# Ecogenomics/CheckM

Measured on NVIDIA H100. Metric: genomes/hour, higher is better.
Workload: dtype int16 (SSV) / u8 (MSV) / int16 (Viterbi) / f32 (Forward, domain definition)

## Files before the change

### checkm_b200/csrc/kernels_vitp.cu

```cuda
#include "engine.hpp"
#include "device_utils.cuh"
#include "stages.hpp"

namespace ckm {

constexpr uint32_t VP_FLOORW = 0xD800D800u;
constexpr int      VP_FLOOR  = -10240;
constexpr uint32_t VP_TFLOORW = 0xC000C000u;

__device__ __forceinline__ int vp_lo(uint32_t w) { return (int)(int16_t)(w & 0xffffu); }
__device__ __forceinline__ int vp_hi(uint32_t w) { return (int)w >> 16; }

template <int W, bool TSMEM>
__global__ void __launch_bounds__(128) vitp_kernel(FilterParams p, int cls) {
  extern __shared__ __align__(16) uint8_t vsm[];
  const int lane = threadIdx.x & 31, warp = threadIdx.x >> 5, wpb = blockDim.x >> 5;
  uint4 *tws = reinterpret_cast<uint4 *>(vsm) + (size_t)warp * W * 64;
  const uint32_t sel = (lane == 0) ? 0x1054u : 0x3210u;
  const int n = min(*p.in_count, p.in_cap);
  int32_t *cursor = (p.vit_work != nullptr) ? p.vit_work + cls : nullptr;
  for (int64_t it = 0;; ++it) {
    int64_t base64;
    if (cursor != nullptr) {
      int b = 0;
      if (lane == 0) b = atomicAdd(cursor, 32);
      base64 = __shfl_sync(0xffffffffu, b, 0);
    } else {
      base64 = ((it * gridDim.x + blockIdx.x) * wpb + warp) * 32;
    }
    if (base64 >= n) break;
    const int base = (int)base64;
    bool mine = false;
    if (base + lane < n) {
      const int vq = p.ms[p.in[base + lane].model].vq;
      mine = (vq == 2 * W) || (W == 1 && vq == 0);
    }
    unsigned todo = __ballot_sync(0xffffffffu, mine);
  while (todo != 0u) {
    const int c = base + __ffs(todo) - 1;
    todo &= todo - 1u;
    Candidate cd = p.in[c];
    const int m = cd.model;
    const ModelScalars ms = p.ms[m];
    const bool unclassed = (ms.vq == 0 && W == 1);
    if (ms.vq != 2 * W && !unclassed) continue;
    const int s = cd.seq, L = p.len[s];
    bool pass = true, redo = false;
    if (cd.P > p.F2) {
      const int tmove = p.tmove_w[s];
      const int cost = -tmove - (int)ms.vit_tbm + 64;
      const bool c1 = (cost - (int)ms.xw_e_loop <= 22528) && (cost <= 22240);
      const bool c1p = (cost - (int)ms.xw_e_loop <= 16384);
      redo = unclassed || !c1;
      float vsc = 0.0f;
      if (!redo) {
        uint4 tr0[TSMEM ? 1 : W], tr1[TSMEM ? 1 : W];
        const uint4 *tsrc = p.twp + ms.blk_off * 32;
        if (TSMEM) {
          __syncwarp();
          for (int z = lane; z < W * 64; z += 32) tws[(z & 1) * (W * 32) + (z >> 1)] = __ldg(tsrc + z);
          __syncwarp();
        } else {
#pragma unroll
          for (int w = 0; w < W; ++w) { tr0[TSMEM ? 0 : w] = __ldg(tsrc + (w * 32 + lane) * 2); tr1[TSMEM ? 0 : w] = __ldg(tsrc + (w * 32 + lane) * 2 + 1); }
        }
#define TR0(w) (TSMEM ? tws[(w) * 32 + lane] : tr0[TSMEM ? 0 : (w)])
#define TR1(w) (TSMEM ? tws[W * 32 + (w) * 32 + lane] : tr1[TSMEM ? 0 : (w)])
        const uint32_t *rwp = p.rwp + ms.blk_off * 32 * (KPAD / 2) + lane;
        uint32_t Mx[W], Ix[W], Dx[W];
#pragma unroll
        for (int w = 0; w < W; ++w) { Mx[w] = VP_FLOORW; Ix[w] = VP_FLOORW; Dx[w] = VP_FLOORW; }
        const int ddbound = ms.ddbound_w, cap = 32767 - (int)ms.vit_emax;
        const int e_move = ms.xw_e_move, e_loop = ms.xw_e_loop;
        int xN = ms.base_w, xB = xN + tmove, xJ = -32768, xC = -32768;
        const uint4 *rp = reinterpret_cast<const uint4 *>(p.res + p.off[s]);
        const int nblk = (L + 15) >> 4;
        uint4 r16 = (nblk > 0) ? __ldg(rp) : make_uint4(0, 0, 0, 0);
        uint32_t ecur[W];
        {
          const uint32_t x0 = r16.x & 0xffu;
#pragma unroll
          for (int w = 0; w < W; ++w) ecur[w] = __ldg(rwp + (x0 * W + w) * 32);
        }
        bool stop = false;
        for (int b = 0; b < nblk && !stop; ++b) {
          const uint4 rnext = (b + 1 < nblk) ? __ldg(rp + b + 1) : make_uint4(0, 0, 0, 0);
          for (int j = 0; j < 4 && !stop; ++j) {
            const uint32_t wcur = (j == 0) ? r16.x : (j == 1) ? r16.y : (j == 2) ? r16.z : r16.w;
            const uint32_t wnxt = (j == 0) ? r16.y : (j == 1) ? r16.z : (j == 2) ? r16.w : rnext.x;
#pragma unroll
            for (int rr = 0; rr < 4; ++rr) {
              if (b * 16 + j * 4 + rr >= L) { stop = true; break; }
              uint32_t enext[W];
              {
                const uint32_t xn = (rr < 3) ? ((wcur >> (8 * (rr + 1))) & 0xffu) : (wnxt & 0xffu);
#pragma unroll
                for (int w = 0; w < W; ++w) enext[w] = __ldg(rwp + (xn * W + w) * 32);
              }
              const uint32_t shM = __shfl_sync(0xffffffffu, Mx[W - 1], (lane + 31) & 31);
              const uint32_t shI = __shfl_sync(0xffffffffu, Ix[W - 1], (lane + 31) & 31);
              const uint32_t shD = __shfl_sync(0xffffffffu, Dx[W - 1], (lane + 31) & 31);
              const uint32_t pm0 = __byte_perm(shM, VP_FLOORW, sel), pi0 = __byte_perm(shI, VP_FLOORW, sel), pd0 = __byte_perm(shD, VP_FLOORW, sel);
              const uint32_t xBw = __byte_perm((uint32_t)xB, 0u, 0x1010u);
              uint32_t md[W];
              uint32_t xEw = VP_FLOORW, dmw = VP_FLOORW;
#pragma unroll
              for (int w = W - 1; w >= 0; --w) {
                const uint32_t pm = (w > 0) ? Mx[w - 1] : pm0, pi = (w > 0) ? Ix[w - 1] : pi0, pd = (w > 0) ? Dx[w - 1] : pd0;
                const uint4 t0 = TR0(w), t1 = TR1(w);
                uint32_t sv = __viaddmax_s16x2(xBw, t0.x, VP_FLOORW);
                sv = __viaddmax_s16x2(pm, t0.y, sv);
                sv = __viaddmax_s16x2(pi, t0.z, sv);
                sv = __viaddmax_s16x2(pd, t0.w, sv);
                sv = __viaddmax_s16x2(sv, ecur[w], VP_FLOORW);
                const uint32_t nI = __viaddmax_s16x2(Ix[w], t1.z, __viaddmax_s16x2(Mx[w], t1.y, VP_FLOORW));
                md[w] = __viaddmax_s16x2(sv, t1.x, VP_FLOORW);
                Mx[w] = sv; Ix[w] = nI;
              }
#pragma unroll
              for (int w = 0; w + 1 < W; w += 2) { xEw = __vimax3_s16x2(xEw, Mx[w], Mx[w + 1]); dmw = __vimax3_s16x2(dmw, md[w], md[w + 1]); }
              if (W & 1) { xEw = __vimax3_s16x2(xEw, Mx[W - 1], Mx[W - 1]); dmw = __vimax3_s16x2(dmw, md[W - 1], md[W - 1]); }
              const int xE = __reduce_max_sync(0xffffffffu, max(vp_lo(xEw), vp_hi(xEw)));
              if (xE >= cap) { redo = true; stop = true; break; }
              xC = max(xC, xE + e_move);
              xJ = max(xJ, xE + e_loop);
              xB = max(xJ + tmove, xN + tmove);
              const int Dmax = __reduce_max_sync(0xffffffffu, max(vp_lo(dmw), vp_hi(dmw)));
              if (Dmax + ddbound > xB) {
                if (!c1p) { redo = true; stop = true; break; }
                uint32_t Bb = VP_FLOORW, Tb = 0u;
#pragma unroll
                for (int w = 0; w < W; ++w) { const uint32_t tdd = TR1(w).w; Bb = __viaddmax_s16x2(Bb, tdd, md[w]); Tb = __viaddmax_s16x2(Tb, __vimax3_s16x2(tdd, VP_TFLOORW, VP_TFLOORW), VP_TFLOORW); }
                uint32_t Bs = Bb, Ts = Tb;
#pragma unroll
                for (int o = 1; o < 32; o <<= 1) {
                  const uint32_t Bl = __shfl_up_sync(0xffffffffu, Bs, o), Tl = __shfl_up_sync(0xffffffffu, Ts, o);
                  if (lane >= o) { Bs = __viaddmax_s16x2(Bl, Ts, Bs); Ts = __viaddmax_s16x2(Ts, Tl, VP_TFLOORW); }
                }
                uint32_t din = __shfl_up_sync(0xffffffffu, Bs, 1), Tex = __shfl_up_sync(0xffffffffu, Ts, 1);
                if (lane == 0) { din = VP_FLOORW; Tex = 0u; }
                const uint32_t lowexit = __shfl_sync(0xffffffffu, Bs, 31);
                const uint32_t dmid = __byte_perm(lowexit, VP_FLOORW, 0x1054u);
                din = __viaddmax_s16x2(dmid, Tex, din);
                uint32_t d = din;
#pragma unroll
                for (int w = 0; w < W; ++w) { Dx[w] = d; d = __viaddmax_s16x2(d, TR1(w).w, md[w]); }
              } else {
                const uint32_t shd = __shfl_sync(0xffffffffu, md[W - 1], (lane + 31) & 31);
#pragma unroll
                for (int w = W - 1; w >= 1; --w) Dx[w] = md[w - 1];
                Dx[0] = __byte_perm(shd, VP_FLOORW, sel);
              }
#pragma unroll
              for (int w = 0; w < W; ++w) ecur[w] = enext[w];
            }
          }
          r16 = rnext;
        }
        if (!redo && xC <= VP_FLOOR + e_move) redo = true;
        if (!redo) {
          vsc = __fsub_rn(__fadd_rn((float)xC, (float)tmove), (float)ms.base_w);
          vsc = __fdiv_rn(vsc, ms.scale_w);
          vsc = __fsub_rn(vsc, 3.0f);
        }
#undef TR0
#undef TR1
      }
      if (redo) {
        if (lane == 0) {
          const int pos = atomicAdd(p.redo_count, 1);
          if (pos < p.redo_cap) p.redo[pos] = cd;
        }
        continue;
      }
      cd.vitsc = vsc;
      const float seq_score = __fdiv_rn(__fsub_rn(vsc, cd.filtersc), 0.69314718055994529f);
      const double P = gumbel_surv((double)seq_score, (double)ms.evparam[2], (double)ms.evparam[3]);
      cd.P = P;
      pass = (P <= p.F2);
      if (lane == 0 && p.dense_vit != nullptr) p.dense_vit[(int64_t)p.model_slot[m] * p.nseq + s] = vsc;
    }
    if (lane == 0 && pass) {
      const int pos = atomicAdd(p.out_count, 1);
      if (pos < p.out_cap) p.out[pos] = cd;
      if (p.dense_passed != nullptr) atomicOr_u8(p.dense_passed, (int64_t)p.model_slot[m] * p.nseq + s, 4);
    }
  }
  }
}

template <int W, bool TSMEM>
static int launch_vitp_w(const FilterParams &p, int cls, int grid, cudaStream_t st) {
  const int sm = TSMEM ? 4 * W * 64 * (int)sizeof(uint4) : 0;
  if (sm > 48 * 1024) {
    cudaError_t e = cudaFuncSetAttribute(vitp_kernel<W, TSMEM>, cudaFuncAttributeMaxDynamicSharedMemorySize, sm);
    if (e != cudaSuccess) return cuda_fail(e, "cudaFuncSetAttribute(vitp)");
  }
  vitp_kernel<W, TSMEM><<<grid, 128, sm, st>>>(p, cls);
  cudaError_t e = cudaGetLastError();
  return e == cudaSuccess ? CKM_OK : cuda_fail(e, "vitp_kernel launch");
}

__global__ void all_pairs_kernel(Candidate *out, int32_t *count, const int32_t *slot_model, int32_t nslots, int32_t nseq) {
  const int64_t n = (int64_t)nslots * nseq;
  for (int64_t i = blockIdx.x * (int64_t)blockDim.x + threadIdx.x; i < n; i += (int64_t)gridDim.x * blockDim.x) {
    Candidate cd;
    cd.seq = (int32_t)(i % nseq); cd.model = slot_model[i / nseq]; cd.usc = 0.0f; cd.filtersc = 0.0f; cd.vitsc = 0.0f; cd.fwdsc = 0.0f; cd.P = 1.0;
    out[i] = cd;
  }
  if (blockIdx.x == 0 && threadIdx.x == 0) *count = (int32_t)n;
}
int launch_all_pairs(Candidate *out, int32_t *count, const int32_t *slot_model, int32_t nslots, int32_t nseq, cudaStream_t st) {
  all_pairs_kernel<<<592, 256, 0, st>>>(out, count, slot_model, nslots, nseq);
  cudaError_t e = cudaGetLastError();
  return e == cudaSuccess ? CKM_OK : cuda_fail(e, "all_pairs_kernel launch");
}

int launch_vitp(const FilterParams &p, int cls, int grid, cudaStream_t st) {
  switch (cls) {
    case 0: return launch_vitp_w<1, false>(p, cls, grid, st);
    case 1: return launch_vitp_w<2, false>(p, cls, grid, st);
    case 2: return launch_vitp_w<3, false>(p, cls, grid, st);
    case 3: return launch_vitp_w<4, false>(p, cls, grid, st);
    case 4: return launch_vitp_w<6, true>(p, cls, grid, st);
    case 5: return launch_vitp_w<8, true>(p, cls, grid, st);
    case 6: return launch_vitp_w<10, true>(p, cls, grid, st);
    case 7: return launch_vitp_w<12, true>(p, cls, grid, st);
    case 8: return launch_vitp_w<14, true>(p, cls, grid, st);
    case 9: return launch_vitp_w<16, true>(p, cls, grid, st);
  }
  set_error("launch_vitp: bad class"); return CKM_EINVAL;
// ... 4 lines not shown
```

### checkm_b200/csrc/search.cu

```cuda
#include <algorithm>
#include <atomic>
#include <chrono>
#include <cstdio>
#include <cmath>
#include <cstdlib>
#include <cstring>
#include <memory>
#include <vector>
#include "engine.hpp"
#include "stages.hpp"
#include "pool.hpp"

using namespace ckm;

namespace ckm {

std::atomic<int> g_live_engines{0};
thread_local ckm_engine *g_pool_engine = nullptr;
thread_local int g_pool_next = 0;
constexpr int X_NX_HOST = 6;
struct EnsembleJob;
int ensembles_launch(ckm_engine *e, const ckm_models *m, DomdefParams &p, const std::vector<PairWork> &pairs,
                     const std::vector<Region> &regs, const std::vector<int> &multi_idx, const std::vector<EnsembleCaps> &caps,
                     cudaStream_t st, EnsembleJob **job_out);
// ... 230 lines not shown
  for (int c = 0; c < 4; ++c) {
    if (gl[c].empty() || db->nseq == 0) continue;
    sp.group_list = s1.glist.as<int32_t>() + goff[c]; sp.ngroups = (int32_t)gl[c].size();
    sp.unit_counter = e->d_counters + CTR_UNIT4 + c;
    int64_t maxbytes = 0;
    for (int g : gl[c]) maxbytes = std::max<int64_t>(maxbytes, m->groups[g].table_bytes);
    const int64_t units = (int64_t)sp.ngroups * sp.nchunks;
    const int grid = (int)std::min<int64_t>(nsm, units);
    if ((rc = launch_ssv(Js[c], sp, grid, (size_t)maxbytes, st))) return rc;
    e->stats.kernel_launches++;
  }
  if (!m->ssv_bypass.empty()) {
    if ((rc = launch_ssv_bypass(m->d_ssv_bypass, (int32_t)m->ssv_bypass.size(), db->nseq, db->d_len, db->d_bin,
                                am.all_active ? nullptr : am.model_active.as<uint8_t>(), (int32_t)m->models.size(),
                                s1.cand.as<int2>(), e->d_counters + CTR_CAND, s1.cand_cap, st))) return rc;
    e->stats.kernel_launches++;
  }
  CKM_CUDA(cudaEventRecord(e->ev[EV_MSV], st));
  MsvParams p{};
  p.res = db->d_res; p.off = db->d_off; p.len = db->d_len; p.nullsc = db->d_nullsc; p.tjb = db->d_tjb;
  p.ms = m->d_scalars; p.rbv = m->d_rbv; p.rmb = m->d_rmb;
  p.cand = s1.cand.as<int2>(); p.cand_count = e->d_counters + CTR_CAND; p.cand_cap = s1.cand_cap;
  p.out = s1.pass.as<Candidate>(); p.out_count = e->d_counters + CTR_MSV; p.out_cap = s1.pass_cap;
  p.xj_dense = xj_dense; p.model_slot = am.model_slot.as<int32_t>(); p.nseq = db->nseq;
  p.row_bytes = (m->maxM + 2 + 15) / 16 * 16;
  p.F1 = 0.02;
  p.use_blk = k.blk ? 1 : 0;
  if ((rc = per_class(e, p, launch_msv2, 16, launch_msv_exact, 4))) return rc;
  e->stats.kernel_launches += 1 + (p.use_blk ? N_BLK_CLASSES : 0);
  CKM_CUDA(cudaEventRecord(e->ev[EV_BIAS], st));
  return CKM_OK;
}

static int run_viterbi(ckm_engine *e, FilterParams &p, bool packed) {
  int rc;
  if (packed) {
    p.vit_work = e->d_counters + CTR_VWORK;
    if ((rc = per_class<FilterParams>(e, p, launch_vitp, 8, nullptr, 0))) return rc;
    p.in = p.redo; p.in_count = p.redo_count; p.in_cap = p.redo_cap;
  }
  return per_class(e, p, launch_vit2, 8, launch_vit, 4);
}
struct Stage2 {
  DevBuf a, b, redo;
  int32_t cap = 0;
};
static int run_stage2(ckm_engine *e, const SearchKnobs &k, const ckm_models *m, const ckm_seqdb *db, ActiveMasks &am, Stage1 &s1, Stage2 &s2,
                      float *d_filtersc, float *d_vit, float *d_fwd, uint8_t *d_passed) {
  cudaStream_t st = e->stream;
  int rc;
  s2.cap = s1.pass_cap;
  if ((rc = s2.a.alloc(sizeof(Candidate) * (size_t)s2.cap))) return rc;
  if ((rc = s2.b.alloc(sizeof(Candidate) * (size_t)s2.cap))) return rc;
  if ((rc = s2.redo.alloc(sizeof(Candidate) * (size_t)s2.cap))) return rc;
  const int nsm = e->prop.multiProcessorCount;
  FilterParams p = filter_params(m, db, am);
  p.redo = s2.redo.as<Candidate>(); p.redo_count = e->d_counters + CTR_VREDO; p.redo_cap = s2.cap;
  p.use_blk = k.blk ? 1 : 0;
  p.dense_filtersc = d_filtersc; p.dense_vit = d_vit; p.dense_fwd = d_fwd; p.dense_passed = d_passed;
  p.in = s1.pass.as<Candidate>(); p.in_count = e->d_counters + CTR_MSV; p.in_cap = s1.pass_cap;
  p.out = s2.a.as<Candidate>(); p.out_count = e->d_counters + CTR_BIAS; p.out_cap = s2.cap;
  if ((rc = launch_bias(p, nsm * 8, st))) return rc;
  CKM_CUDA(cudaEventRecord(e->ev[EV_VIT], st));
  p.in = s2.a.as<Candidate>(); p.in_count = e->d_counters + CTR_BIAS; p.in_cap = s2.cap;
  p.out = s2.b.as<Candidate>(); p.out_count = e->d_counters + CTR_VIT; p.out_cap = s2.cap;
  if ((rc = run_viterbi(e, p, k.vitp))) return rc;
  CKM_CUDA(cudaEventRecord(e->ev[EV_FWD], st));
  p.in = s2.b.as<Candidate>(); p.in_count = e->d_counters + CTR_VIT; p.in_cap = s2.cap;
  p.out = s2.a.as<Candidate>(); p.out_count = e->d_counters + CTR_FWD; p.out_cap = s2.cap;
  if ((rc = per_class(e, p, launch_fwd2, 8, launch_fwd, 4, true))) return rc;
  CKM_CUDA(cudaEventRecord(e->ev[EV_CASCADE_END], st));
  e->stats.kernel_launches += 3 + (k.vitp ? N_BLK_CLASSES : 0) + (p.use_blk ? 2 * N_BLK_CLASSES : 0);
  return CKM_OK;
}

static int64_t envelope_need(const ckm_models *m, const PairWork &pw, const Envelope &en, bool use_blk) {
  const int64_t Ld = en.j - en.i + 1, Mpad = ((m->models[pw.model].M + 1) + 31) / 32 * 32 + 32;
  const int64_t vq = use_blk ? vq_of(m->models[pw.model].M) : 0;
  const int64_t width = vq ? 32 * vq : Mpad;
  return (vq ? 1 : 2) * (Ld + 1) * 3 * width + (Ld + 1) * 15 + 64;
}
static int run_envelope_waves(ckm_engine *e, const ckm_models *m, const std::vector<PairWork> &pairs, DomdefParams &p, int64_t budget,
                              DevBuf &scratch, std::vector<Envelope> &ev, DevBuf &d_ev, DevBuf &d_ord, bool leave_last) {
  if (ev.empty()) return CKM_OK;
  cudaStream_t st = e->stream;
  int rc;
  std::vector<int64_t> need(ev.size());
  std::vector<int8_t> ecls(ev.size());
  for (size_t i = 0; i < ev.size(); ++i) {
    const PairWork &pw = pairs[ev[i].pair];
    need[i] = envelope_need(m, pw, ev[i], p.use_blk != 0);
    ecls[i] = (int8_t)cls_of(m->models[pw.model].M, p.use_blk != 0);
  }
  budget = std::max<int64_t>(budget, *std::max_element(need.begin(), need.end()));
  if ((rc = d_ev.alloc(sizeof(Envelope) * ev.size())) || (rc = d_ord.alloc(sizeof(int32_t) * ev.size()))) return rc;
  std::vector<int32_t> eorder(ev.size());
  for (size_t w0 = 0, w1; w0 < ev.size(); w0 = w1) {
    int64_t tot = 0;
    for (w1 = w0; w1 < ev.size() && (w1 == w0 || tot + need[w1] <= budget); ++w1) { ev[w1].scratch_off = tot; tot += need[w1]; }
// ... 451 lines not shown
  if ((rc = run_stage1(e, k, m, db, q.am, n, s1, nullptr))) return rc;
  if ((rc = run_stage2(e, k, m, db, q.am, s1, s2, dfs.as<float>(), dvit.as<float>(), dfwd.as<float>(), dpass.as<uint8_t>()))) return rc;
  int32_t ctr[CTR_N];
  CKM_CUDA(cudaMemcpyAsync(ctr, e->d_counters, sizeof(ctr), cudaMemcpyDeviceToHost, e->stream));
  CKM_CUDA(cudaMemcpyAsync(filtersc_out, dfs.p, sizeof(float) * (size_t)n, cudaMemcpyDeviceToHost, e->stream));
  CKM_CUDA(cudaMemcpyAsync(vit_out, dvit.p, sizeof(float) * (size_t)n, cudaMemcpyDeviceToHost, e->stream));
  CKM_CUDA(cudaMemcpyAsync(fwd_out, dfwd.p, sizeof(float) * (size_t)n, cudaMemcpyDeviceToHost, e->stream));
  CKM_CUDA(cudaMemcpyAsync(passed_out, dpass.p, (size_t)n, cudaMemcpyDeviceToHost, e->stream));
  CKM_CUDA(cudaStreamSynchronize(e->stream));
  if (ctr[CTR_CAND] > s1.cand_cap || ctr[CTR_MSV] > s1.pass_cap) { set_error("candidate queue overflow"); return CKM_ECAPACITY; }
  std::vector<Candidate> pass1((size_t)ctr[CTR_MSV]);
  if (!pass1.empty()) CKM_CUDA(cudaMemcpy(pass1.data(), s1.pass.p, sizeof(Candidate) * pass1.size(), cudaMemcpyDeviceToHost));
  for (const Candidate &c : pass1) passed_out[(int64_t)q.qorder[0][c.model] * db->nseq + c.seq] |= 1;
  fill_filter_stats(e, n, ctr,  0, 5);
  return CKM_OK;
}

int ckm_viterbi_scores(ckm_engine *e, const ckm_models *m, const int32_t *model_idx, int32_t nmodels,
                       const ckm_seqdb *db, int32_t mode, float *vit_out) {
  if (!e || !m || !db || !vit_out) { set_error("ckm_viterbi_scores: bad argument"); return CKM_EINVAL; }
  cudaSetDevice(e->device);
  cudaStream_t st = e->stream;
  const int ndb = (int)m->models.size();
  if (model_idx == nullptr) nmodels = ndb;
  const int64_t n = (int64_t)nmodels * db->nseq;
  if (n > ((int64_t)1 << 30)) { set_error("ckm_viterbi_scores: too many pairs for one call"); return CKM_ECAPACITY; }
  PoolScope pool_scope(e);
  ActiveMasks am; std::vector<int32_t> slot;
  int rc = build_masks(m, db, model_idx, nmodels, nullptr, am, slot, st);
  if (rc) return rc;
  std::vector<int32_t> slot_model((size_t)std::max(nmodels, 1));
  for (int i = 0; i < nmodels; ++i) slot_model[i] = model_idx ? model_idx[i] : i;
  const size_t nf = (size_t)std::max<int64_t>(n, 1);
  DevBuf dsm, din, dout, dredo, dvit;
  if ((rc = dsm.alloc(sizeof(int32_t) * slot_model.size())) || (rc = din.alloc(sizeof(Candidate) * nf)) || (rc = dout.alloc(sizeof(Candidate) * nf)) ||
      (rc = dredo.alloc(sizeof(Candidate) * nf)) || (rc = dvit.alloc(sizeof(float) * nf))) return rc;
  CKM_CUDA(cudaMemcpyAsync(dsm.p, slot_model.data(), sizeof(int32_t) * slot_model.size(), cudaMemcpyHostToDevice, st));
  CKM_CUDA(cudaMemsetAsync(e->d_counters, 0, CTR_N * sizeof(int32_t), st));
  CKM_CUDA(cudaMemsetAsync(dvit.p, 0xff, sizeof(float) * nf, st));
  std::memset(&e->stats, 0, sizeof(e->stats));
  if (n > 0) {
    if ((rc = launch_all_pairs(din.as<Candidate>(), e->d_counters + CTR_BIAS, dsm.as<int32_t>(), nmodels, db->nseq, st))) return rc;
    FilterParams p = filter_params(m, db, am);
    p.use_blk = (mode == 2) ? 0 : 1;
    p.dense_vit = dvit.as<float>();
    p.redo = dredo.as<Candidate>(); p.redo_count = e->d_counters + CTR_VREDO; p.redo_cap = (int32_t)nf;
    p.in = din.as<Candidate>(); p.in_count = e->d_counters + CTR_BIAS; p.in_cap = (int32_t)nf;
    p.out = dout.as<Candidate>(); p.out_count = e->d_counters + CTR_VIT; p.out_cap = (int32_t)nf;
    if ((rc = run_viterbi(e, p, mode == 0))) return rc;
  }
  int32_t ctr[CTR_N];
  CKM_CUDA(cudaMemcpyAsync(ctr, e->d_counters, sizeof(ctr), cudaMemcpyDeviceToHost, st));
  CKM_CUDA(cudaMemcpyAsync(vit_out, dvit.p, sizeof(float) * (size_t)n, cudaMemcpyDeviceToHost, st));
  CKM_CUDA(cudaStreamSynchronize(st));
  e->stats.n_pairs = n; e->stats.n_past_bias = ctr[CTR_BIAS]; e->stats.n_past_vit = ctr[CTR_VIT]; e->stats.n_vit_redo = ctr[CTR_VREDO];
  return CKM_OK;
}

int ckm_msv_scores(ckm_engine *e, const ckm_models *m, const int32_t *model_idx, int32_t nmodels,
                   const ckm_seqdb *db, int32_t *xj_out) {
  if (!e || !m || !db || !xj_out) { set_error("ckm_msv_scores: bad argument"); return CKM_EINVAL; }
  cudaSetDevice(e->device);
  const SearchKnobs k = read_knobs(false);
  PoolScope pool_scope(e);
  QueryPlan q;
  int rc = plan_queries(m, db, model_idx, nmodels, nullptr, q, e->stream);
  if (rc) return rc;
  const int64_t n = q.n_pairs;
  DevBuf dense;
  if ((rc = dense.alloc(sizeof(int32_t) * (size_t)std::max<int64_t>(n, 1)))) return rc;
  CKM_CUDA(cudaMemsetAsync(dense.p, 0xff, sizeof(int32_t) * (size_t)n, e->stream));
  Stage1 s1;
  std::memset(&e->stats, 0, sizeof(e->stats));
  if ((rc = run_stage1(e, k, m, db, q.am, n, s1, dense.as<int32_t>()))) return rc;
  int32_t ctr[CTR_N];
  CKM_CUDA(cudaMemcpyAsync(ctr, e->d_counters, sizeof(ctr), cudaMemcpyDeviceToHost, e->stream));
  unsigned long long cells = 0;
  CKM_CUDA(cudaMemcpyAsync(&cells, s1.cells.p, sizeof(cells), cudaMemcpyDeviceToHost, e->stream));
  CKM_CUDA(cudaMemcpyAsync(xj_out, dense.p, sizeof(int32_t) * (size_t)n, cudaMemcpyDeviceToHost, e->stream));
  CKM_CUDA(cudaStreamSynchronize(e->stream));
  if (ctr[CTR_CAND] > s1.cand_cap || ctr[CTR_MSV] > s1.pass_cap) { set_error("candidate queue overflow"); return CKM_ECAPACITY; }
  fill_filter_stats(e, n, ctr, cells, 2);
// ... 5 lines not shown
```

### checkm_b200/csrc/stages.hpp

```cpp
#pragma once
#include "engine.hpp"

namespace ckm {

#ifndef CKM_SSV_WARPS
#define CKM_SSV_WARPS 16
#endif
constexpr int SSV_WARPS = CKM_SSV_WARPS;
constexpr int SSV_WARPS_HOST = SSV_WARPS;
constexpr int MSV_WARPS = 8;

struct SsvParams {
  const uint8_t *res; const int64_t *off; const int32_t *len; const int32_t *bin;
  const float *msvB; const int32_t *tjb; const int32_t *order;
  int32_t nseq, seq_chunk, nchunks;
  const TileGroup *groups; const int32_t *group_list; int32_t ngroups;
  const TileDesc *tiles; const TileModel *tile_models;
  const int32_t *chain_first_tile, *chain_ntiles;
  const uint8_t *tile_blob;
  const uint8_t *tile_active;
  const uint8_t *model_active;
  int32_t ntiles, nmodels;
  int32_t *unit_counter;
  int2 *cand; int32_t *cand_count; int32_t cand_cap;
// ... 10 lines not shown
int launch_ssv(int J, const SsvParams &p, int grid, size_t smem_bytes, cudaStream_t stream);

struct MsvParams {
  const uint8_t *res; const int64_t *off; const int32_t *len;
  const float *nullsc; const int32_t *tjb;
  const ModelScalars *ms; const uint8_t *rbv; const uint32_t *rmb;
  const int2 *cand; const int32_t *cand_count; int32_t cand_cap;
  Candidate *out; int32_t *out_count; int32_t out_cap;
  int32_t *xj_dense;
  const int32_t *model_slot;
  int32_t nseq;
  int32_t row_bytes;
  int32_t use_blk;
  double F1;
};

int launch_msv_exact(const MsvParams &p, int grid, cudaStream_t stream);
int launch_ssv_bypass(const int32_t *models, int32_t nbypass, int32_t nseq, const int32_t *len, const int32_t *bin,
                      const uint8_t *model_active, int32_t nmodels_db, int2 *cand, int32_t *cand_count, int32_t cand_cap,
                      cudaStream_t stream);
int launch_msv2(const MsvParams &p, int cls, int grid, cudaStream_t stream);

constexpr int VIT_WARPS = 4;
constexpr int FWD_WARPS = 4;
struct FilterParams {
  const uint8_t *res; const int64_t *off; const int32_t *len;
  const float *lenA, *lenB;
  const int16_t *tmove_w;
  const ModelScalars *ms;
  const float *bias_eo; const int16_t *rwv; const int16_t *twv; const float *rfv; const float *tfv;
  const uint4 *twb; const uint32_t *rwb; const float4 *tfb; const float *rfb;
  const uint4 *twp; const uint32_t *rwp;
  Candidate *redo; int32_t *redo_count; int32_t redo_cap;
  int32_t *vit_work;
  const Candidate *in; const int32_t *in_count; int32_t in_cap;
  Candidate *out; int32_t *out_count; int32_t out_cap;
  int32_t row_elems;
  double F1, F2, F3;
  int32_t use_blk;
  float *dense_filtersc, *dense_vit, *dense_fwd; uint8_t *dense_passed;
  const int32_t *model_slot; int32_t nseq;
};
int launch_bias(const FilterParams &p, int grid, cudaStream_t st);
int launch_vit(const FilterParams &p, int grid, cudaStream_t st);
constexpr int N_BLK_CLASSES = 10;
constexpr int BLK_Q[N_BLK_CLASSES] = {2, 4, 6, 8, 12, 16, 20, 24, 28, 32};
int launch_vit2(const FilterParams &p, int cls, int grid, cudaStream_t st);
int launch_vitp(const FilterParams &p, int cls, int grid, cudaStream_t st);
int launch_all_pairs(Candidate *out, int32_t *count, const int32_t *slot_model, int32_t nslots, int32_t nseq, cudaStream_t st);
int launch_fwd(const FilterParams &p, int grid, cudaStream_t st);

#define FLT_MIN_F 1.17549435e-38f
struct PairWork {
  int32_t seq, model, L;
  int32_t first_dom, ndom_slots;
  float   fwdsc, filtersc, usc;
  int64_t row_off;
};
struct Region { int32_t pair, i, j, multi; };
constexpr int ENS_MAXENV = 32;
struct EnsembleCaps { int32_t segments, trace_segments, envelopes; };
constexpr EnsembleCaps ENS_DEFAULT_CAPS = {4096, 64, ENS_MAXENV};
struct Envelope { int32_t pair, i, j, null2_done; int64_t scratch_off; int32_t slot, pad; };
struct DomainOut {
  int32_t pair, ienv, jenv, hmmfrom, hmmto, sqfrom, sqto, ok;
  float   envsc, domcorrection, oasc, bitscore, dombias, pad;
  double  lnP;
};
struct HitOut { float pre_score, score, sum_score; int32_t ndom, valid, pad; double lnP; };
struct DomdefParams {
  const uint8_t *res; const int64_t *off; const float *nullsc;
  const ModelScalars *ms; const float *rfv; const float *tfv;
  const PairWork *pairs; int32_t npairs;
  const int32_t *pair_order; int32_t pair_begin, pair_end;
  float *xf, *xb, *btot, *etot, *mocc, *n2sc;
  int32_t *trace;
  Region *regions; int32_t *region_count; int32_t region_cap;
  const Envelope *envs; const int32_t *env_order; int32_t env_begin, env_end;
  float *scratch;
  DomainOut *doms; HitOut *hits;
  const float *logsum_tbl;
// ... 13 lines not shown
```

Baseline: 33870.

## Group Viterbi candidates by model and stage emission tables in shared memory

Adds count/scan/scatter kernels that bucket Viterbi candidates by model and class into chunks of up to 64. Each block claims one chunk and loads that model's emission and transition tables into shared memory once. Its warps then pull candidates from the chunk through a shared atomic counter. This replaces per-row global __ldg emission lookups and per-candidate table reloads with shared-memory reads, at the cost of three extra kernel launches, more shared memory per block (which may lower occupancy), and block-level synchronisation.

```diff
diff --git a/checkm_b200/csrc/kernels_vitp.cu b/checkm_b200/csrc/kernels_vitp.cu
--- a/checkm_b200/csrc/kernels_vitp.cu
+++ b/checkm_b200/csrc/kernels_vitp.cu
@@ -11,151 +11,222 @@
 __device__ __forceinline__ int vp_lo(uint32_t w) { return (int)(int16_t)(w & 0xffffu); }
 __device__ __forceinline__ int vp_hi(uint32_t w) { return (int)w >> 16; }
 
+__device__ __forceinline__ void vit_pass(const FilterParams &p, const Candidate &cd) {
+  const int pos = atomicAdd(p.out_count, 1);
+  if (pos < p.out_cap) p.out[pos] = cd;
+  if (p.dense_passed != nullptr) atomicOr_u8(p.dense_passed, (int64_t)p.model_slot[cd.model] * p.nseq + cd.seq, 4);
+}
+__device__ __forceinline__ void vit_redo(const FilterParams &p, const Candidate &cd) {
+  const int pos = atomicAdd(p.redo_count, 1);
+  if (pos < p.redo_cap) p.redo[pos] = cd;
+}
+__device__ __forceinline__ int vitp_class(int vq) { return vq == 0 ? -1 : (vq <= 8 ? vq / 2 - 1 : vq / 4 + 1); }
+
+__global__ void vit_count_kernel(FilterParams p, int32_t *cnt) {
+  const int n = min(*p.in_count, p.in_cap);
+  for (int i = blockIdx.x * blockDim.x + threadIdx.x; i < n; i += gridDim.x * blockDim.x) {
+    const Candidate cd = p.in[i];
+    if (!(cd.P > p.F2)) vit_pass(p, cd);
+    else if (p.ms[cd.model].vq == 0) vit_redo(p, cd);
+    else atomicAdd(cnt + cd.model, 1);
+  }
+}
+
+__global__ void __launch_bounds__(1024) vit_scan_kernel(FilterParams p, int32_t nmodels, const int32_t *cnt, int32_t *off, int32_t *choff) {
+  __shared__ int ws[2][32];
+  const int lane = threadIdx.x & 31, warp = threadIdx.x >> 5;
+  int run_pairs = 0, run_chunks = 0;
+  for (int c = 0; c < N_BLK_CLASSES; ++c) {
+    if (threadIdx.x == 0) p.vit_cls_chunks[c] = run_chunks;
+    for (int b = 0; b < nmodels; b += 1024) {
+      const int m = b + threadIdx.x;
+      const int v = (m < nmodels && vitp_class(p.ms[m].vq) == c) ? cnt[m] : 0, h = (v + VITP_CHUNK - 1) / VITP_CHUNK;
+      int sv = v, sh = h;
+#pragma unroll
+      for (int o = 1; o < 32; o <<= 1) {
+        const int a = __shfl_up_sync(0xffffffffu, sv, o), d = __shfl_up_sync(0xffffffffu, sh, o);
+        if (lane >= o) { sv += a; sh += d; }
+      }
+      if (lane == 31) { ws[0][warp] = sv; ws[1][warp] = sh; }
+      __syncthreads();
+      if (warp == 0) {
+        int tv = ws[0][lane], th = ws[1][lane];
+#pragma unroll
+        for (int o = 1; o < 32; o <<= 1) {
+          const int a = __shfl_up_sync(0xffffffffu, tv, o), d = __shfl_up_sync(0xffffffffu, th, o);
+          if (lane >= o) { tv += a; th += d; }
+        }
+        ws[0][lane] = tv; ws[1][lane] = th;
+      }
+      __syncthreads();
+      if (v > 0) {
+        off[m] = run_pairs + (warp ? ws[0][warp - 1] : 0) + sv - v;
+        choff[m] = run_chunks + (warp ? ws[1][warp - 1] : 0) + sh - h;
+      }
+      run_pairs += ws[0][31]; run_chunks += ws[1][31];
+      __syncthreads();
+    }
+  }
+  if (threadIdx.x == 0) p.vit_cls_chunks[N_BLK_CLASSES] = run_chunks;
+}
+
+__global__ void vit_scatter_kernel(FilterParams p, const int32_t *cnt, int32_t *fill, const int32_t *off, const int32_t *choff) {
+  const int n = min(*p.in_count, p.in_cap);
+  for (int i = blockIdx.x * blockDim.x + threadIdx.x; i < n; i += gridDim.x * blockDim.x) {
+    const int m = p.in[i].model;
+    if (!(p.in[i].P > p.F2) || p.ms[m].vq == 0) continue;
+    const int r = atomicAdd(fill + m, 1), pos = off[m] + r;
+    p.vit_idx[pos] = i;
+    if (r % VITP_CHUNK == 0) p.vit_chunks[choff[m] + r / VITP_CHUNK] = make_int2(pos, off[m] + min(r + VITP_CHUNK, cnt[m]));
+  }
+}
+
+int launch_vit_group(const FilterParams &p, int32_t nmodels, int32_t *ws, int grid, cudaStream_t st) {
+  int32_t *cnt = ws, *fill = ws + nmodels, *off = ws + 2 * (size_t)nmodels, *choff = ws + 3 * (size_t)nmodels;
+  cudaError_t e = cudaMemsetAsync(ws, 0, sizeof(int32_t) * 2 * (size_t)nmodels, st);
+  if (e != cudaSuccess) return cuda_fail(e, "cudaMemsetAsync(vit groups)");
+  vit_count_kernel<<<grid, 256, 0, st>>>(p, cnt);
+  vit_scan_kernel<<<1, 1024, 0, st>>>(p, nmodels, cnt, off, choff);
+  vit_scatter_kernel<<<grid, 256, 0, st>>>(p, cnt, fill, off, choff);
+  e = cudaGetLastError();
+  return e == cudaSuccess ? CKM_OK : cuda_fail(e, "vit grouping launch");
+}
+
+constexpr int VITP_THREADS = 128;
+
+__host__ __device__ constexpr int vitp_smem_bytes(int W, bool tsmem) { return KPAD * W * 32 * 4 + (tsmem ? W * 64 * 16 : 0); }
+__host__ __device__ constexpr int vitp_min_blocks(int W) { return W <= 4 ? 4 : (W <= 10 ? 3 : 2); }
+
 template <int W, bool TSMEM>
-__global__ void __launch_bounds__(128) vitp_kernel(FilterParams p, int cls) {
-  extern __shared__ __align__(16) uint8_t vsm[];
-  const int lane = threadIdx.x & 31, warp = threadIdx.x >> 5, wpb = blockDim.x >> 5;
-  uint4 *tws = reinterpret_cast<uint4 *>(vsm) + (size_t)warp * W * 64;
+__global__ void __launch_bounds__(VITP_THREADS, vitp_min_blocks(W)) vitp_kernel(FilterParams p, int cls) {
+  extern __shared__ __align__(16) uint4 vsm[];
+  __shared__ int s_chunk, s_next;
+  __shared__ ModelScalars s_ms;
+  uint32_t *esm = reinterpret_cast<uint32_t *>(vsm);
+  uint4 *tws = vsm + KPAD * W * 8;
+  const int lane = threadIdx.x & 31;
   const uint32_t sel = (lane == 0) ? 0x1054u : 0x3210u;
-  const int n = min(*p.in_count, p.in_cap);
-  int32_t *cursor = (p.vit_work != nullptr) ? p.vit_work + cls : nullptr;
-  for (int64_t it = 0;; ++it) {
-    int64_t base64;
-    if (cursor != nullptr) {
-      int b = 0;
-      if (lane == 0) b = atomicAdd(cursor, 32);
-      base64 = __shfl_sync(0xffffffffu, b, 0);
-    } else {
-      base64 = ((it * gridDim.x + blockIdx.x) * wpb + warp) * 32;
-    }
-    if (base64 >= n) break;
-    const int base = (int)base64;
-    bool mine = false;
-    if (base + lane < n) {
-      const int vq = p.ms[p.in[base + lane].model].vq;
-      mine = (vq == 2 * W) || (W == 1 && vq == 0);
-    }
-    unsigned todo = __ballot_sync(0xffffffffu, mine);
-  while (todo != 0u) {
-    const int c = base + __ffs(todo) - 1;
-    todo &= todo - 1u;
-    Candidate cd = p.in[c];
-    const int m = cd.model;
-    const ModelScalars ms = p.ms[m];
-    const bool unclassed = (ms.vq == 0 && W == 1);
-    if (ms.vq != 2 * W && !unclassed) continue;
-    const int s = cd.seq, L = p.len[s];
-    bool pass = true, redo = false;
-    if (cd.P > p.F2) {
+  const int c0 = p.vit_cls_chunks[cls], nch = p.vit_cls_chunks[cls + 1] - c0;
+  for (;;) {
+    __syncthreads();
+    if (threadIdx.x == 0) {
+      const int k = atomicAdd(p.vit_work + cls, 1);
+      s_chunk = k;
+      if (k < nch) {
+        s_next = p.vit_chunks[c0 + k].x;
+        s_ms = p.ms[p.in[p.vit_idx[s_next]].model];
+      }
+    }
+    __syncthreads();
+    const int k = s_chunk;
+    if (k >= nch) break;
+    const int2 ch = p.vit_chunks[c0 + k];
+    const ModelScalars &ms = s_ms;
+    {
+      const uint4 *esrc = reinterpret_cast<const uint4 *>(p.rwp + ms.blk_off * 32 * (KPAD / 2));
+      for (int z = threadIdx.x; z < KPAD * W * 8; z += VITP_THREADS) vsm[z] = __ldg(esrc + z);
+      if (TSMEM) {
+        const uint4 *tsrc = p.twp + ms.blk_off * 32;
+        for (int z = threadIdx.x; z < W * 64; z += VITP_THREADS) tws[(z & 1) * (W * 32) + (z >> 1)] = __ldg(tsrc + z);
+      }
+    }
+    uint4 tr0[TSMEM ? 1 : W], tr1[TSMEM ? 1 : W];
+    if (!TSMEM) {
+      const uint4 *tsrc = p.twp + ms.blk_off * 32;
+#pragma unroll
+      for (int w = 0; w < W; ++w) { tr0[TSMEM ? 0 : w] = __ldg(tsrc + (w * 32 + lane) * 2); tr1[TSMEM ? 0 : w] = __ldg(tsrc + (w * 32 + lane) * 2 + 1); }
+    }
+#define TR0(w) (TSMEM ? tws[(w) * 32 + lane] : tr0[TSMEM ? 0 : (w)])
+#define TR1(w) (TSMEM ? tws[W * 32 + (w) * 32 + lane] : tr1[TSMEM ? 0 : (w)])
+    __syncthreads();
+    const uint32_t *erow = esm + lane;
+    const int ddbound = ms.ddbound_w, cap = 32767 - (int)ms.vit_emax;
+    const int e_move = ms.xw_e_move, e_loop = ms.xw_e_loop;
+    for (;;) {
+      int j = 0;
+      if (lane == 0) j = atomicAdd(&s_next, 1);
+      j = __shfl_sync(0xffffffffu, j, 0);
+      if (j >= ch.y) break;
+      const Candidate *cin = p.in + p.vit_idx[j];
+      const int s = cin->seq, L = p.len[s];
+      bool redo = false;
       const int tmove = p.tmove_w[s];
       const int cost = -tmove - (int)ms.vit_tbm + 64;
       const bool c1 = (cost - (int)ms.xw_e_loop <= 22528) && (cost <= 22240);
       const bool c1p = (cost - (int)ms.xw_e_loop <= 16384);
-      redo = unclassed || !c1;
+      redo = !c1;
       float vsc = 0.0f;
       if (!redo) {
-        uint4 tr0[TSMEM ? 1 : W], tr1[TSMEM ? 1 : W];
-        const uint4 *tsrc = p.twp + ms.blk_off * 32;
-        if (TSMEM) {
-          __syncwarp();
-          for (int z = lane; z < W * 64; z += 32) tws[(z & 1) * (W * 32) + (z >> 1)] = __ldg(tsrc + z);
-          __syncwarp();
-        } else {
-#pragma unroll
-          for (int w = 0; w < W; ++w) { tr0[TSMEM ? 0 : w] = __ldg(tsrc + (w * 32 + lane) * 2); tr1[TSMEM ? 0 : w] = __ldg(tsrc + (w * 32 + lane) * 2 + 1); }
-        }
-#define TR0(w) (TSMEM ? tws[(w) * 32 + lane] : tr0[TSMEM ? 0 : (w)])
-#define TR1(w) (TSMEM ? tws[W * 32 + (w) * 32 + lane] : tr1[TSMEM ? 0 : (w)])
-        const uint32_t *rwp = p.rwp + ms.blk_off * 32 * (KPAD / 2) + lane;
         uint32_t Mx[W], Ix[W], Dx[W];
 #pragma unroll
         for (int w = 0; w < W; ++w) { Mx[w] = VP_FLOORW; Ix[w] = VP_FLOORW; Dx[w] = VP_FLOORW; }
-        const int ddbound = ms.ddbound_w, cap = 32767 - (int)ms.vit_emax;
-        const int e_move = ms.xw_e_move, e_loop = ms.xw_e_loop;
         int xN = ms.base_w, xB = xN + tmove, xJ = -32768, xC = -32768;
-        const uint4 *rp = reinterpret_cast<const uint4 *>(p.res + p.off[s]);
-        const int nblk = (L + 15) >> 4;
-        uint4 r16 = (nblk > 0) ? __ldg(rp) : make_uint4(0, 0, 0, 0);
-        uint32_t ecur[W];
-        {
-          const uint32_t x0 = r16.x & 0xffu;
-#pragma unroll
-          for (int w = 0; w < W; ++w) ecur[w] = __ldg(rwp + (x0 * W + w) * 32);
-        }
+        const uint32_t *rp = reinterpret_cast<const uint32_t *>(p.res + p.off[s]);
+        const int nw = (L + 3) >> 2;
+        uint32_t wcur = (nw > 0) ? __ldg(rp) : 0u;
         bool stop = false;
-        for (int b = 0; b < nblk && !stop; ++b) {
-          const uint4 rnext = (b + 1 < nblk) ? __ldg(rp + b + 1) : make_uint4(0, 0, 0, 0);
-          for (int j = 0; j < 4 && !stop; ++j) {
-            const uint32_t wcur = (j == 0) ? r16.x : (j == 1) ? r16.y : (j == 2) ? r16.z : r16.w;
-            const uint32_t wnxt = (j == 0) ? r16.y : (j == 1) ? r16.z : (j == 2) ? r16.w : rnext.x;
-#pragma unroll
-            for (int rr = 0; rr < 4; ++rr) {
-              if (b * 16 + j * 4 + rr >= L) { stop = true; break; }
-              uint32_t enext[W];
-              {
-                const uint32_t xn = (rr < 3) ? ((wcur >> (8 * (rr + 1))) & 0xffu) : (wnxt & 0xffu);
-#pragma unroll
-                for (int w = 0; w < W; ++w) enext[w] = __ldg(rwp + (xn * W + w) * 32);
+        for (int q = 0; q < nw && !stop; ++q) {
+          const uint32_t wnext = (q + 1 < nw) ? __ldg(rp + q + 1) : 0u;
+#pragma unroll
+          for (int rr = 0; rr < 4; ++rr) {
+            if (q * 4 + rr >= L) { stop = true; break; }
+            const uint32_t *ew = erow + ((wcur >> (8 * rr)) & 0xffu) * (W * 32);
+            const uint32_t shM = __shfl_sync(0xffffffffu, Mx[W - 1], (lane + 31) & 31);
+            const uint32_t shI = __shfl_sync(0xffffffffu, Ix[W - 1], (lane + 31) & 31);
+            const uint32_t shD = __shfl_sync(0xffffffffu, Dx[W - 1], (lane + 31) & 31);
+            const uint32_t pm0 = __byte_perm(shM, VP_FLOORW, sel), pi0 = __byte_perm(shI, VP_FLOORW, sel), pd0 = __byte_perm(shD, VP_FLOORW, sel);
+            const uint32_t xBw = __byte_perm((uint32_t)xB, 0u, 0x1010u);
+            uint32_t md[W];
+            uint32_t xEw = VP_FLOORW, dmw = VP_FLOORW;
+#pragma unroll
+            for (int w = W - 1; w >= 0; --w) {
+              const uint32_t pm = (w > 0) ? Mx[w - 1] : pm0, pi = (w > 0) ? Ix[w - 1] : pi0, pd = (w > 0) ? Dx[w - 1] : pd0;
+              const uint4 t0 = TR0(w), t1 = TR1(w);
+              uint32_t sv = __viaddmax_s16x2(xBw, t0.x, VP_FLOORW);
+              sv = __viaddmax_s16x2(pm, t0.y, sv);
+              sv = __viaddmax_s16x2(pi, t0.z, sv);
+              sv = __viaddmax_s16x2(pd, t0.w, sv);
+              sv = __viaddmax_s16x2(sv, ew[w * 32], VP_FLOORW);
+              const uint32_t nI = __viaddmax_s16x2(Ix[w], t1.z, __viaddmax_s16x2(Mx[w], t1.y, VP_FLOORW));
+              md[w] = __viaddmax_s16x2(sv, t1.x, VP_FLOORW);
+              Mx[w] = sv; Ix[w] = nI;
+            }
+#pragma unroll
+            for (int w = 0; w + 1 < W; w += 2) { xEw = __vimax3_s16x2(xEw, Mx[w], Mx[w + 1]); dmw = __vimax3_s16x2(dmw, md[w], md[w + 1]); }
+            if (W & 1) { xEw = __vimax3_s16x2(xEw, Mx[W - 1], Mx[W - 1]); dmw = __vimax3_s16x2(dmw, md[W - 1], md[W - 1]); }
+            const int xE = __reduce_max_sync(0xffffffffu, max(vp_lo(xEw), vp_hi(xEw)));
+            if (xE >= cap) { redo = true; stop = true; break; }
+            xC = max(xC, xE + e_move);
+            xJ = max(xJ, xE + e_loop);
+            xB = max(xJ + tmove, xN + tmove);
+            const int Dmax = __reduce_max_sync(0xffffffffu, max(vp_lo(dmw), vp_hi(dmw)));
+            if (Dmax + ddbound > xB) {
+              if (!c1p) { redo = true; stop = true; break; }
+              uint32_t Bb = VP_FLOORW, Tb = 0u;
+#pragma unroll
+              for (int w = 0; w < W; ++w) { const uint32_t tdd = TR1(w).w; Bb = __viaddmax_s16x2(Bb, tdd, md[w]); Tb = __viaddmax_s16x2(Tb, __vimax3_s16x2(tdd, VP_TFLOORW, VP_TFLOORW), VP_TFLOORW); }
+              uint32_t Bs = Bb, Ts = Tb;
+#pragma unroll
+              for (int o = 1; o < 32; o <<= 1) {
+                const uint32_t Bl = __shfl_up_sync(0xffffffffu, Bs, o), Tl = __shfl_up_sync(0xffffffffu, Ts, o);
+                if (lane >= o) { Bs = __viaddmax_s16x2(Bl, Ts, Bs); Ts = __viaddmax_s16x2(Ts, Tl, VP_TFLOORW); }
               }
-              const uint32_t shM = __shfl_sync(0xffffffffu, Mx[W - 1], (lane + 31) & 31);
-              const uint32_t shI = __shfl_sync(0xffffffffu, Ix[W - 1], (lane + 31) & 31);
-              const uint32_t shD = __shfl_sync(0xffffffffu, Dx[W - 1], (lane + 31) & 31);
-              const uint32_t pm0 = __byte_perm(shM, VP_FLOORW, sel), pi0 = __byte_perm(shI, VP_FLOORW, sel), pd0 = __byte_perm(shD, VP_FLOORW, sel);
-              const uint32_t xBw = __byte_perm((uint32_t)xB, 0u, 0x1010u);
-              uint32_t md[W];
-              uint32_t xEw = VP_FLOORW, dmw = VP_FLOORW;
-#pragma unroll
-              for (int w = W - 1; w >= 0; --w) {
-                const uint32_t pm = (w > 0) ? Mx[w - 1] : pm0, pi = (w > 0) ? Ix[w - 1] : pi0, pd = (w > 0) ? Dx[w - 1] : pd0;
-                const uint4 t0 = TR0(w), t1 = TR1(w);
-                uint32_t sv = __viaddmax_s16x2(xBw, t0.x, VP_FLOORW);
-                sv = __viaddmax_s16x2(pm, t0.y, sv);
-                sv = __viaddmax_s16x2(pi, t0.z, sv);
-                sv = __viaddmax_s16x2(pd, t0.w, sv);
-                sv = __viaddmax_s16x2(sv, ecur[w], VP_FLOORW);
-                const uint32_t nI = __viaddmax_s16x2(Ix[w], t1.z, __viaddmax_s16x2(Mx[w], t1.y, VP_FLOORW));
-                md[w] = __viaddmax_s16x2(sv, t1.x, VP_FLOORW);
-                Mx[w] = sv; Ix[w] = nI;
-              }
-#pragma unroll
-              for (int w = 0; w + 1 < W; w += 2) { xEw = __vimax3_s16x2(xEw, Mx[w], Mx[w + 1]); dmw = __vimax3_s16x2(dmw, md[w], md[w + 1]); }
-              if (W & 1) { xEw = __vimax3_s16x2(xEw, Mx[W - 1], Mx[W - 1]); dmw = __vimax3_s16x2(dmw, md[W - 1], md[W - 1]); }
-              const int xE = __reduce_max_sync(0xffffffffu, max(vp_lo(xEw), vp_hi(xEw)));
-              if (xE >= cap) { redo = true; stop = true; break; }
-              xC = max(xC, xE + e_move);
-              xJ = max(xJ, xE + e_loop);
-              xB = max(xJ + tmove, xN + tmove);
-              const int Dmax = __reduce_max_sync(0xffffffffu, max(vp_lo(dmw), vp_hi(dmw)));
-              if (Dmax + ddbound > xB) {
-                if (!c1p) { redo = true; stop = true; break; }
-                uint32_t Bb = VP_FLOORW, Tb = 0u;
-#pragma unroll
-                for (int w = 0; w < W; ++w) { const uint32_t tdd = TR1(w).w; Bb = __viaddmax_s16x2(Bb, tdd, md[w]); Tb = __viaddmax_s16x2(Tb, __vimax3_s16x2(tdd, VP_TFLOORW, VP_TFLOORW), VP_TFLOORW); }
-                uint32_t Bs = Bb, Ts = Tb;
-#pragma unroll
-                for (int o = 1; o < 32; o <<= 1) {
-                  const uint32_t Bl = __shfl_up_sync(0xffffffffu, Bs, o), Tl = __shfl_up_sync(0xffffffffu, Ts, o);
-                  if (lane >= o) { Bs = __viaddmax_s16x2(Bl, Ts, Bs); Ts = __viaddmax_s16x2(Ts, Tl, VP_TFLOORW); }
-                }
-                uint32_t din = __shfl_up_sync(0xffffffffu, Bs, 1), Tex = __shfl_up_sync(0xffffffffu, Ts, 1);
-                if (lane == 0) { din = VP_FLOORW; Tex = 0u; }
-                const uint32_t lowexit = __shfl_sync(0xffffffffu, Bs, 31);
-                const uint32_t dmid = __byte_perm(lowexit, VP_FLOORW, 0x1054u);
-                din = __viaddmax_s16x2(dmid, Tex, din);
-                uint32_t d = din;
-#pragma unroll
-                for (int w = 0; w < W; ++w) { Dx[w] = d; d = __viaddmax_s16x2(d, TR1(w).w, md[w]); }
-              } else {
-                const uint32_t shd = __shfl_sync(0xffffffffu, md[W - 1], (lane + 31) & 31);
-#pragma unroll
-                for (int w = W - 1; w >= 1; --w) Dx[w] = md[w - 1];
-                Dx[0] = __byte_perm(shd, VP_FLOORW, sel);
-              }
-#pragma unroll
-              for (int w = 0; w < W; ++w) ecur[w] = enext[w];
+              uint32_t din = __shfl_up_sync(0xffffffffu, Bs, 1), Tex = __shfl_up_sync(0xffffffffu, Ts, 1);
+              if (lane == 0) { din = VP_FLOORW; Tex = 0u; }
+              const uint32_t lowexit = __shfl_sync(0xffffffffu, Bs, 31);
+              const uint32_t dmid = __byte_perm(lowexit, VP_FLOORW, 0x1054u);
+              din = __viaddmax_s16x2(dmid, Tex, din);
+              uint32_t d = din;
+#pragma unroll
+              for (int w = 0; w < W; ++w) { Dx[w] = d; d = __viaddmax_s16x2(d, TR1(w).w, md[w]); }
+            } else {
+              const uint32_t shd = __shfl_sync(0xffffffffu, md[W - 1], (lane + 31) & 31);
+#pragma unroll
+              for (int w = W - 1; w >= 1; --w) Dx[w] = md[w - 1];
+              Dx[0] = __byte_perm(shd, VP_FLOORW, sel);
             }
           }
-          r16 = rnext;
+          wcur = wnext;
         }
         if (!redo && xC <= VP_FLOOR + e_move) redo = true;
         if (!redo) {
@@ -163,40 +234,34 @@
           vsc = __fdiv_rn(vsc, ms.scale_w);
           vsc = __fsub_rn(vsc, 3.0f);
         }
-#undef TR0
-#undef TR1
-      }
+      }
+      Candidate cd = *cin;
       if (redo) {
-        if (lane == 0) {
-          const int pos = atomicAdd(p.redo_count, 1);
-          if (pos < p.redo_cap) p.redo[pos] = cd;
-        }
+        if (lane == 0) vit_redo(p, cd);
         continue;
       }
       cd.vitsc = vsc;
       const float seq_score = __fdiv_rn(__fsub_rn(vsc, cd.filtersc), 0.69314718055994529f);
       const double P = gumbel_surv((double)seq_score, (double)ms.evparam[2], (double)ms.evparam[3]);
       cd.P = P;
-      pass = (P <= p.F2);
-      if (lane == 0 && p.dense_vit != nullptr) p.dense_vit[(int64_t)p.model_slot[m] * p.nseq + s] = vsc;
-    }
-    if (lane == 0 && pass) {
-      const int pos = atomicAdd(p.out_count, 1);
-      if (pos < p.out_cap) p.out[pos] = cd;
-      if (p.dense_passed != nullptr) atomicOr_u8(p.dense_passed, (int64_t)p.model_slot[m] * p.nseq + s, 4);
-    }
-  }
+      if (lane == 0) {
+        if (p.dense_vit != nullptr) p.dense_vit[(int64_t)p.model_slot[cd.model] * p.nseq + s] = vsc;
+        if (P <= p.F2) vit_pass(p, cd);
+      }
+    }
+#undef TR0
+#undef TR1
   }
 }
 
 template <int W, bool TSMEM>
 static int launch_vitp_w(const FilterParams &p, int cls, int grid, cudaStream_t st) {
-  const int sm = TSMEM ? 4 * W * 64 * (int)sizeof(uint4) : 0;
+  constexpr int sm = vitp_smem_bytes(W, TSMEM);
   if (sm > 48 * 1024) {
     cudaError_t e = cudaFuncSetAttribute(vitp_kernel<W, TSMEM>, cudaFuncAttributeMaxDynamicSharedMemorySize, sm);
     if (e != cudaSuccess) return cuda_fail(e, "cudaFuncSetAttribute(vitp)");
   }
-  vitp_kernel<W, TSMEM><<<grid, 128, sm, st>>>(p, cls);
+  vitp_kernel<W, TSMEM><<<grid, VITP_THREADS, sm, st>>>(p, cls);
   cudaError_t e = cudaGetLastError();
   return e == cudaSuccess ? CKM_OK : cuda_fail(e, "vitp_kernel launch");
 }
diff --git a/checkm_b200/csrc/search.cu b/checkm_b200/csrc/search.cu
--- a/checkm_b200/csrc/search.cu
+++ b/checkm_b200/csrc/search.cu
@@ -286,17 +286,27 @@
   return CKM_OK;
 }
 
-static int run_viterbi(ckm_engine *e, FilterParams &p, bool packed) {
+static int run_viterbi(ckm_engine *e, const ckm_models *m, FilterParams &p, bool packed, DevBuf &grp) {
   int rc;
   if (packed) {
+    const int nm = (int)m->models.size();
+    const size_t nchunks = (size_t)p.in_cap / VITP_CHUNK + nm + 1;
+    const size_t words = 4 * (size_t)nm + 16 + ((size_t)p.in_cap + 1) / 2 * 2;
+    if ((rc = grp.alloc(sizeof(int32_t) * words + sizeof(int2) * nchunks))) return rc;
+    int32_t *ws = grp.as<int32_t>();
+    p.vit_cls_chunks = ws + 4 * (size_t)nm;
+    p.vit_idx = p.vit_cls_chunks + 16;
+    p.vit_chunks = reinterpret_cast<int2 *>(ws + words);
     p.vit_work = e->d_counters + CTR_VWORK;
+    if ((rc = launch_vit_group(p, nm, ws, e->prop.multiProcessorCount * 8, e->stream))) return rc;
     if ((rc = per_class<FilterParams>(e, p, launch_vitp, 8, nullptr, 0))) return rc;
+    e->stats.kernel_launches += 3;
     p.in = p.redo; p.in_count = p.redo_count; p.in_cap = p.redo_cap;
   }
   return per_class(e, p, launch_vit2, 8, launch_vit, 4);
 }
 struct Stage2 {
-  DevBuf a, b, redo;
+  DevBuf a, b, redo, vgrp;
   int32_t cap = 0;
 };
 static int run_stage2(ckm_engine *e, const SearchKnobs &k, const ckm_models *m, const ckm_seqdb *db, ActiveMasks &am, Stage1 &s1, Stage2 &s2,
@@ -318,7 +328,7 @@
   CKM_CUDA(cudaEventRecord(e->ev[EV_VIT], st));
   p.in = s2.a.as<Candidate>(); p.in_count = e->d_counters + CTR_BIAS; p.in_cap = s2.cap;
   p.out = s2.b.as<Candidate>(); p.out_count = e->d_counters + CTR_VIT; p.out_cap = s2.cap;
-  if ((rc = run_viterbi(e, p, k.vitp))) return rc;
+  if ((rc = run_viterbi(e, m, p, k.vitp, s2.vgrp))) return rc;
   CKM_CUDA(cudaEventRecord(e->ev[EV_FWD], st));
   p.in = s2.b.as<Candidate>(); p.in_count = e->d_counters + CTR_VIT; p.in_cap = s2.cap;
   p.out = s2.a.as<Candidate>(); p.out_count = e->d_counters + CTR_FWD; p.out_cap = s2.cap;
@@ -836,7 +846,7 @@
   std::vector<int32_t> slot_model((size_t)std::max(nmodels, 1));
   for (int i = 0; i < nmodels; ++i) slot_model[i] = model_idx ? model_idx[i] : i;
   const size_t nf = (size_t)std::max<int64_t>(n, 1);
-  DevBuf dsm, din, dout, dredo, dvit;
+  DevBuf dsm, din, dout, dredo, dvit, dgrp;
   if ((rc = dsm.alloc(sizeof(int32_t) * slot_model.size())) || (rc = din.alloc(sizeof(Candidate) * nf)) || (rc = dout.alloc(sizeof(Candidate) * nf)) ||
       (rc = dredo.alloc(sizeof(Candidate) * nf)) || (rc = dvit.alloc(sizeof(float) * nf))) return rc;
   CKM_CUDA(cudaMemcpyAsync(dsm.p, slot_model.data(), sizeof(int32_t) * slot_model.size(), cudaMemcpyHostToDevice, st));
@@ -851,7 +861,7 @@
     p.redo = dredo.as<Candidate>(); p.redo_count = e->d_counters + CTR_VREDO; p.redo_cap = (int32_t)nf;
     p.in = din.as<Candidate>(); p.in_count = e->d_counters + CTR_BIAS; p.in_cap = (int32_t)nf;
     p.out = dout.as<Candidate>(); p.out_count = e->d_counters + CTR_VIT; p.out_cap = (int32_t)nf;
-    if ((rc = run_viterbi(e, p, mode == 0))) return rc;
+    if ((rc = run_viterbi(e, m, p, mode == 0, dgrp))) return rc;
   }
   int32_t ctr[CTR_N];
   CKM_CUDA(cudaMemcpyAsync(ctr, e->d_counters, sizeof(ctr), cudaMemcpyDeviceToHost, st));
diff --git a/checkm_b200/csrc/stages.hpp b/checkm_b200/csrc/stages.hpp
--- a/checkm_b200/csrc/stages.hpp
+++ b/checkm_b200/csrc/stages.hpp
@@ -66,7 +66,7 @@
   const uint4 *twb; const uint32_t *rwb; const float4 *tfb; const float *rfb;
   const uint4 *twp; const uint32_t *rwp;
   Candidate *redo; int32_t *redo_count; int32_t redo_cap;
-  int32_t *vit_work;
+  int32_t *vit_idx; int2 *vit_chunks; int32_t *vit_cls_chunks; int32_t *vit_work;
   const Candidate *in; const int32_t *in_count; int32_t in_cap;
   Candidate *out; int32_t *out_count; int32_t out_cap;
   int32_t row_elems;
@@ -81,6 +81,8 @@
 constexpr int BLK_Q[N_BLK_CLASSES] = {2, 4, 6, 8, 12, 16, 20, 24, 28, 32};
 int launch_vit2(const FilterParams &p, int cls, int grid, cudaStream_t st);
 int launch_vitp(const FilterParams &p, int cls, int grid, cudaStream_t st);
+constexpr int VITP_CHUNK = 64;
+int launch_vit_group(const FilterParams &p, int32_t nmodels, int32_t *ws, int grid, cudaStream_t st);
 int launch_all_pairs(Candidate *out, int32_t *count, const int32_t *slot_model, int32_t nslots, int32_t nseq, cudaStream_t st);
 int launch_fwd(const FilterParams &p, int grid, cudaStream_t st);
 
```

After: 35520 (median of 6 runs). +4.9%, better.
